# ntampellini/FIRECODE

Hardware: AMD Instinct MI355X
Metric: conformer-pair RMSD alignments/s (higher is better)
Workload: dtype f64

## Files before the change

firecode_amd/csrc/fc_kabsch.hip:

```cpp
#include <type_traits>

#include "fc_internal.h"
#include <vector>
#include "fc_kabsch_math.h"

#include <algorithm>
#include <cstdlib>

namespace fc {

__global__ void __launch_bounds__(256)
k_prep(const double *__restrict__ coords, int64_t N, int64_t A_all, const int32_t *__restrict__ sel,
       int64_t A, int center, int64_t Npad, double *__restrict__ Xs, double *__restrict__ G,
       double *__restrict__ Xa, unsigned long long *__restrict__ gmax_bits,
       const int32_t *__restrict__ conf_idx) {
  const int64_t n = (int64_t)blockIdx.x * blockDim.x + threadIdx.x;
  if (n >= Npad) return;
  for (int64_t a = A; a < ((A + 3) & ~(int64_t)3); ++a) {
    Xs[(a * 3 + 0) * Npad + n] = 0.0;
    Xs[(a * 3 + 1) * Npad + n] = 0.0;
    Xs[(a * 3 + 2) * Npad + n] = 0.0;
  }
  if (n >= N) {
    for (int64_t a = 0; a < A; ++a) {
// ... 430 lines not shown
    push_pairs(m, may, i, j, pairq, Q, counters, lane);
  }
}

__device__ __forceinline__ void flush_pairs_wave32(const uint32_t *__restrict__ sq_wave, int n_staged, unsigned i0, unsigned j0,
                                                   uint64_t *__restrict__ pairq, unsigned long long Q,
                                                   unsigned long long *__restrict__ counters, int lane) {
  if (n_staged == 0) return;
  unsigned long long base = 0;
  if (lane == 0) base = atomicAdd(&counters[6], (unsigned long long)n_staged);
  base = __shfl(base, 0);
  for (int idx = lane; idx < n_staged; idx += 64) {
    const uint32_t e = sq_wave[idx];
    const unsigned long long slot = base + (unsigned long long)idx;
    if (slot < Q) pairq[slot] = ((uint64_t)(i0 + (e >> 6)) << 32) | (uint64_t)(j0 + (e & 63u));
  }
}
template <int WCAP>
__device__ __forceinline__ void stage_pairs_wave32(uint64_t m, bool may, unsigned i, unsigned j, unsigned i0, unsigned j0,
                                                   uint32_t *__restrict__ sq_wave, int &n_staged,
                                                   uint64_t *__restrict__ pairq, unsigned long long Q,
                                                   unsigned long long *__restrict__ counters, int lane) {
  if (m == 0) return;
  const int n = (int)__popcll(m);
  if (n > WCAP) {
    push_pairs(m, may, i, j, pairq, Q, counters, lane);
    return;
  }
  if (n_staged + n > WCAP) {
    flush_pairs_wave32(sq_wave, n_staged, i0, j0, pairq, Q, counters, lane);
    n_staged = 0;
  }
  if (may) sq_wave[n_staged + (int)__popcll(m & ((1ull << lane) - 1ull))] = ((i - i0) << 6) | (j - j0);
  n_staged += n;
}

template <bool USE_LDS, int TI, int NW, bool ENANT = false>
__global__ void __launch_bounds__(NW * 64)
k_simbits_screen(const double *__restrict__ Xs, const double *__restrict__ G, int64_t N,
                 int64_t Npad, int A, double A_thr2, int IB, int64_t rank, int64_t world,
                 uint64_t *__restrict__ bits, int64_t W, uint32_t *__restrict__ cand,
                 unsigned long long *__restrict__ counters, uint64_t *__restrict__ pairq,
                 unsigned long long Q) {
  extern __shared__ double lds[];
  const int tid = threadIdx.x;
  const int lane = tid & 63;
  const int wv = __builtin_amdgcn_readfirstlane(tid >> 6);
  const int64_t jt = blockIdx.x;
  const int64_t lb = blockIdx.y;
  const int64_t gb = global_block(lb, rank, world);
  const int64_t i0 = gb * IB;
  if (i0 >= N) return;
  if (jt * 64 + 63 <= i0) return;
  const int64_t j = jt * 64 + lane;

  if (USE_LDS) {
    const int total = A * 3 * 64;
    for (int idx = tid; idx < total; idx += NW * 64) {
      const int ac = idx >> 6, l = idx & 63;
      lds[idx] = Xs[(int64_t)ac * Npad + jt * 64 + l];
    }
    __syncthreads();
  }
  const double Gq = G[j];
  const double *__restrict__ xq = Xs + jt * 64 + lane;

  for (int it = wv; it * TI < IB; it += NW) {
    const int64_t ib = i0 + (int64_t)it * TI;
    if (ib >= N) break;
    if (jt * 64 + 63 <= ib) break;
    double acc[TI][9];
#pragma unroll
    for (int k = 0; k < TI; ++k)
#pragma unroll
      for (int e = 0; e < 9; ++e) acc[k][e] = 0.0;

    const double *__restrict__ xp = Xs + ib;
#pragma unroll 2
    for (int a = 0; a < A; ++a) {
      double qx, qy, qz;
      if (USE_LDS) {
        qx = lds[(a * 3 + 0) * 64 + lane];
        qy = lds[(a * 3 + 1) * 64 + lane];
        qz = lds[(a * 3 + 2) * 64 + lane];
      } else {
        qx = xq[(int64_t)(a * 3 + 0) * Npad];
        qy = xq[(int64_t)(a * 3 + 1) * Npad];
        qz = xq[(int64_t)(a * 3 + 2) * Npad];
      }
      const double *__restrict__ px = xp + (int64_t)(a * 3 + 0) * Npad;
      const double *__restrict__ py = xp + (int64_t)(a * 3 + 1) * Npad;
      const double *__restrict__ pz = xp + (int64_t)(a * 3 + 2) * Npad;
#pragma unroll
      for (int k = 0; k < TI; ++k) {
        const double x = px[k], y = py[k], z = pz[k];
        acc[k][0] = fma(x, qx, acc[k][0]);
        acc[k][1] = fma(x, qy, acc[k][1]);
        acc[k][2] = fma(x, qz, acc[k][2]);
        acc[k][3] = fma(y, qx, acc[k][3]);
        acc[k][4] = fma(y, qy, acc[k][4]);
        acc[k][5] = fma(y, qz, acc[k][5]);
        acc[k][6] = fma(z, qx, acc[k][6]);
        acc[k][7] = fma(z, qy, acc[k][7]);
        acc[k][8] = fma(z, qz, acc[k][8]);
      }
    }
#pragma unroll
    for (int k = 0; k < TI; ++k) {
      const int64_t i = ib + k;
      const double Gp = G[i];
      bool may = kabsch_may_be_below<ENANT>(acc[k], Gp + Gq, A_thr2);
      may = may && (j > i) && (j < N) && (i < N);
      const uint64_t word = __ballot(may);
      push_pairs(word, may, (unsigned)i, (unsigned)j, pairq, Q, counters, lane);
      if (lane == 0 && i < N) {
        const int64_t lrow = (int64_t)(lb * IB) + (int64_t)it * TI + k;
        bits[lrow * W + jt] = word;
        if (word) {
          const unsigned long long slot = atomicAdd(&counters[4], 1ull);
          cand[slot] = (uint32_t)(lrow * W + jt);
        }
      }
    }
  }
}

typedef double d4_t __attribute__((ext_vector_type(4)));

template <int NW, int MODE = 0, int TC = 64, bool EIG = false, bool ENANT = false>
__global__ void __launch_bounds__(NW * 64, 2)
k_simbits_screen_mfma(const double *__restrict__ Xs, const double *__restrict__ G, int64_t N,
                      int64_t Npad, int A, double A_thr2, int IB, int64_t rank, int64_t world,
                      uint64_t *__restrict__ bits, int64_t W, uint32_t *__restrict__ cand,
                      unsigned long long *__restrict__ counters, uint64_t *__restrict__ pairq,
                      unsigned long long Q, const uint64_t *__restrict__ item_table, unsigned long long n_items,
                      double *__restrict__ rmsd_out = nullptr, const unsigned long long *__restrict__ gate = nullptr,
                      double *__restrict__ maxdev_out = nullptr) {
  static_assert(!EIG || MODE == 2, "EIG: the complete alignments");
  static_assert(!ENANT || MODE == 0, "ENANT: the screen only");
  constexpr bool VALUES = MODE != 0;
  constexpr int NT = MODE == 2 ? 1 : 2;
  static_assert(TC == 64 || ((TC == 32 || TC == 16) && MODE == 2), "column tiles: 64, or 32 / 16 for the complete alignments");
  constexpr int NU = (TC / 16) / NT;
  constexpr int KPR = TC == 64 ? 2 : 4;
  constexpr int SST = 2048 / TC;
  constexpr int CST = TC == 64 ? 256 : 128;
  auto koff = [](int sl) { return TC == 16 ? (sl >> 1) * 384 + (sl & 1) * 64 : sl * (12 * TC); };
  if (gate != nullptr && *gate == 0ull) return;
  extern __shared__ double lds[];
  const int tid = threadIdx.x;
  const int lane = tid & 63;
  const int wv = __builtin_amdgcn_readfirstlane(tid >> 6);
  const int KS = (A + 3) >> 2;
  double *__restrict__ ldsG = lds + (TC == 16 ? ((KS + 1) >> 1) * 384 : KS * 12 * TC);
  uint64_t *__restrict__ stageQ = reinterpret_cast<uint64_t *>(ldsG + TC + IB);
  uint32_t *__restrict__ stageW = reinterpret_cast<uint32_t *>(stageQ + kStagePairs);
  unsigned *__restrict__ stageN = reinterpret_cast<unsigned *>(stageW + kStageWords);
#ifdef FC_TIMELINE
  unsigned long long *tl = MODE == 2 ? reinterpret_cast<unsigned long long *>(bits) : reinterpret_cast<unsigned long long *>(rmsd_out);
  constexpr bool TL = MODE == 0 || MODE == 2;
#endif
  const unsigned long long b = blockIdx.x;
  if (b >= n_items) return;
#ifdef FC_TIMELINE
  if (TL && tl && tid == 0) {
    tl[(size_t)b * 4] = wall_clock64();
    tl[(size_t)b * 4 + 3] = b;
  }
#endif
  int64_t jt, lb;
  int it_first = 0, it_last = IB >> 4;
  if (item_table != nullptr) {
    const uint64_t it = item_table[b];
    lb = item_block(it);
    jt = item_tile(it);
    if constexpr (MODE == 2) it_last = (IB >> 4) * item_blocks(it);
    if (it & kItemFirstHalf) it_last = IB >> 5;
    if (it & kItemSecondHalf) it_first = IB >> 5;
  } else {
    const int64_t NT = Npad / TC;
    jt = (int64_t)(b % (unsigned long long)NT);
    lb = (int64_t)(b / (unsigned long long)NT);
  }
  const int64_t j0 = jt * TC;
  const int64_t i0 = global_block(lb, rank, world) * IB;
  if (i0 >= N) return;
  if (j0 + TC - 1 <= i0) return;
  uint32_t *__restrict__ sq32_wave = reinterpret_cast<uint32_t *>(stageQ) + wv * (kStagePairs * 2 / NW);
  int n_staged32 = 0;
  (void)sq32_wave;
  (void)n_staged32;

  {
    const int n_runs = TC == 64 ? KS * 6 : (TC == 32 ? KS * 3 : ((KS + 1) >> 1) * 3);
    const int cs_l = TC == 64 ? lane >> 4 : lane >> 5, k1_l = TC == 64 ? (lane >> 3) & 1 : (lane >> 3) & 3, c15_l = (lane & 7) * 2;
    for (int q = wv; q < n_runs; q += NW) {
      const int sc = TC == 64 ? q >> 1 : q, kh = TC == 64 ? q & 1 : 0;
      const int sg = sc / 3, c = sc - sg * 3;
      int a = sg * 4 + kh * 2 + k1_l;
      if (TC == 16) {
        a = (sg * 2 + cs_l) * 4 + k1_l;
        a = a < KS * 4 ? a : KS * 4 - 1;
      }
      const double *src = Xs + (int64_t)(a * 3 + c) * Npad + j0 + (TC == 16 ? 0 : cs_l * 16) + c15_l;
      __builtin_amdgcn_global_load_lds((const __attribute__((address_space(1))) void *)src,
                                       (__attribute__((address_space(3))) void *)(lds + q * 128), 16, 0, 0);
    }
    for (int idx = tid; idx < TC + IB; idx += NW * 64) {
      const int64_t g = idx < TC ? j0 + idx : i0 + (idx - TC);
      ldsG[idx] = g < Npad ? G[g] : 0.0;
    }
    if (tid < kStagePairs) stageQ[tid] = ~0ull;
    if (tid < kStageWords) stageW[tid] = ~0u;
    if (tid < 2) stageN[tid] = 0u;
    __syncthreads();
#ifdef FC_TIMELINE
    if (TL && tl && tid == 0) tl[(size_t)b * 4 + 1] = wall_clock64();
#endif
  }
  const int kq = lane >> 4, l15 = lane & 15;
  const int lcol = MODE == 2 ? 4 * (l15 & 3) + (l15 >> 2) : l15;
  const int boff = (kq / KPR) * 128 + (kq % KPR) * 16 + lcol;
  uint16_t *bits16 = reinterpret_cast<uint16_t *>(bits);

  double a0[3], a1[3], a2[3];
  int pre_it = -1;
  const int tpb = IB >> 4;
  auto tile_row = [&](int it_) -> int64_t {
    if constexpr (MODE == 2) {
      const int k = it_ / tpb;
      return global_block(lb + k, rank, world) * IB + (int64_t)(it_ - k * tpb) * 16;
    } else {
      return i0 + (int64_t)it_ * 16;
    }
  };
  auto row_offsets = [&](int it_, unsigned (&vo)[3]) {
    const int64_t ib_ = tile_row(it_);
#pragma unroll
    for (int c = 0; c < 3; ++c) vo[c] = (unsigned)(((int64_t)(kq * 3 + c) * Npad + ib_ + l15) * 8);
  };
  auto fetch_a_at = [&](double (&a)[3], unsigned (&vo)[3], int sx) {
    const int sl = sx < KS ? sx : KS - 1;
    const char *__restrict__ xs_s = reinterpret_cast<const char *>(Xs + (int64_t)sl * 12 * Npad);
#pragma unroll
    for (int c = 0; c < 3; ++c) {
      asm volatile("" : "+v"(vo[c]));
      a[c] = *reinterpret_cast<const double *>(xs_s + vo[c]);
    }
  };

  for (int it = it_first + wv; it < it_last; it += NW) {
    const int64_t ib = tile_row(it);
    if (ib >= N) break;
    if (j0 + TC - 1 <= ib) break;
    const int64_t lrow0 = lb * IB + (int64_t)it * 16;
    double Gp_row = 0.0;
    if constexpr (MODE == 2) Gp_row = G[ib + l15];
    (void)Gp_row;
    unsigned nz = 0;
    unsigned voff[3];
    row_offsets(it, voff);

#pragma unroll 1
    for (int half = 0; half < NU; ++half) {
      const int cs0 = half * NT;
      if (j0 + (cs0 + NT) * 16 - 1 <= ib) {
        if (!VALUES && lane < 16 && ib + lane < N) {
          bits16[((lrow0 + lane) * W + jt) * 4 + cs0] = 0;
          bits16[((lrow0 + lane) * W + jt) * 4 + cs0 + 1] = 0;
        }
        continue;
      }
      if constexpr (MODE == 2) {
        if (j0 + cs0 * 16 >= N) continue;
      }
      d4_t acc[NT][9];

      const double *__restrict__ lb0 = lds + cs0 * SST + boff;
      double b0[NT][3], b1[NT][3];
      const int KSe = KS;
      auto fetch_a = [&](double (&a)[3], int sx) {
        fetch_a_at(a, voff, sx);
      };
      auto fetch_b = [&](double (&b)[NT][3], int sx) {
        const int sl = sx < KS ? sx : KS - 1;
        const double *__restrict__ lb_s = lb0 + koff(sl);
#pragma unroll
        for (int t = 0; t < NT; ++t)
#pragma unroll
          for (int c = 0; c < 3; ++c) b[t][c] = lb_s[c * CST + t * SST];
      };
      auto mma = [&](const double (&a)[3], const double (&b)[NT][3], auto first_) {
        constexpr bool first = decltype(first_)::value;
#pragma unroll
        for (int x = 0; x < 3; ++x)
#pragma unroll
          for (int y = 0; y < 3; ++y)
#pragma unroll
            for (int t = 0; t < NT; ++t) {
              const d4_t c_in = first ? d4_t{0.0, 0.0, 0.0, 0.0} : acc[t][x * 3 + y];
              acc[t][x * 3 + y] = MODE == 2 ? __builtin_amdgcn_mfma_f64_16x16x4f64(b[t][y], a[x], c_in, 0, 0, 0)
                                            : __builtin_amdgcn_mfma_f64_16x16x4f64(a[x], b[t][y], c_in, 0, 0, 0);
            }
      };
      if (pre_it != it) {
        fetch_a_at(a0, voff, 0);
        fetch_a_at(a1, voff, 1);
        fetch_a_at(a2, voff, 2);
      }
      fetch_b(b0, 0);
      fetch_b(b1, 1);
#define FC_KSTEP(AX, BX, U)             \
  if (sgrp + (U) < KSe) {               \
    mma(AX, BX, std::false_type{});     \
    fetch_a(AX, sgrp + (U) + 3);        \
    fetch_b(BX, sgrp + (U) + 2);        \
  }
      mma(a0, b0, std::true_type{});
      fetch_a(a0, 3);
      fetch_b(b0, 2);
      for (int sgrp = 1; sgrp < KSe; sgrp += 6) {
        FC_KSTEP(a1, b1, 0)
        FC_KSTEP(a2, b0, 1)
        FC_KSTEP(a0, b1, 2)
        FC_KSTEP(a1, b0, 3)
        FC_KSTEP(a2, b1, 4)
        FC_KSTEP(a0, b0, 5)
      }
#undef FC_KSTEP
      {
        const bool same_tile = half < NU - 1 && !(MODE == 2 && j0 + (cs0 + NT) * 16 >= N);
        const int nit = same_tile ? it : it + NW;
        bool more = same_tile;
        if (!same_tile && nit < it_last) {
          const int64_t nib = tile_row(nit);
          more = nib < N && !(j0 + TC - 1 <= nib);
        }
        if (more) {
          unsigned vn[3];
          row_offsets(nit, vn);
          fetch_a_at(a0, vn, 0);
          fetch_a_at(a1, vn, 1);
          fetch_a_at(a2, vn, 2);
          pre_it = nit;
        } else {
          pre_it = -1;
        }
      }
      const int n32 = (int)N, ib32 = (int)ib;
#pragma unroll
      for (int t = 0; t < NT; ++t) {
        const int cs = cs0 + t;
        const int j = (int)j0 + cs * 16 + l15;
        const double Gq = ldsG[cs * 16 + l15];
        uint64_t mr[4] = {0, 0, 0, 0};
        if (MODE == 2) {
          const int i = ib32 + l15;
          const int jb = (int)j0 + cs * 16 + 4 * kq;
          const double Gp = Gp_row;
          double nR[4][9];
          bool ok4[4];
          double msdA4[4] = {0.0, 0.0, 0.0, 0.0};
          {
            double B4[4][9], GG[4], Q44[4][4], nq4[4], lam4[4];
#pragma unroll
            for (int r = 0; r < 4; ++r) {
              GG[r] = Gp + ldsG[cs * 16 + 4 * kq + r];
#pragma unroll
              for (int e = 0; e < 9; ++e) B4[r][e] = acc[t][e][r];
            }
            kabsch_quaternion_qcp_lean4(B4, GG, Q44, nq4, ok4, EIG ? lam4 : nullptr);
            if constexpr (EIG) {
              const double k_small = 2e-10 / (double)A;
#pragma unroll
              for (int r = 0; r < 4; ++r) {
                msdA4[r] = GG[r] - 2.0 * lam4[r];
                if (!(msdA4[r] > k_small * GG[r] * GG[r])) ok4[r] = false, msdA4[r] = 0.0;
              }
            }
#pragma unroll
            for (int r = 0; r < 4; ++r) {
              if (!ok4[r]) Q44[r][0] = 1.0, Q44[r][1] = 0.0, Q44[r][2] = 0.0, Q44[r][3] = 0.0, nq4[r] = 1.0;
              neg_rotation_from_raw_quaternion(Q44[r], nq4[r], nR[r]);
            }
          }
          typedef double d2_t __attribute__((ext_vector_type(2)));
          const double *__restrict__ qcol = lds + cs * SST + 4 * kq;
          const double *__restrict__ prow_u = Xs + ib;
          const unsigned l15u = (unsigned)l15;
          const int n_rounds = (A + 1) >> 1, n_groups = n_rounds >> 1;
          const bool odd_round = (n_rounds & 1) != 0;
          double ssq[4] = {0.0, 0.0, 0.0, 0.0}, mx[4] = {0.0, 0.0, 0.0, 0.0};
          const int64_t Npad3 = 3 * Npad;
          const double *__restrict__ pa0 = prow_u, *__restrict__ pa1 = prow_u + Npad, *__restrict__ pa2 = prow_u + 2 * Npad;
          const double *__restrict__ qg = qcol;
          auto load_pq = [&](auto u_, double (&P)[3], d2_t (&Qv)[3][2]) {
            constexpr int u = decltype(u_)::value;
            const double *__restrict__ ql = qg + (u / KPR) * 128 + (u % KPR) * 16;
#pragma unroll
            for (int c = 0; c < 3; ++c) {
              Qv[c][0] = *reinterpret_cast<const d2_t *>(ql + c * CST);
              Qv[c][1] = *reinterpret_cast<const d2_t *>(ql + c * CST + 2);
            }
            P[0] = pa0[l15u];
            P[1] = pa1[l15u];
            P[2] = pa2[l15u];
            pa0 += Npad3;
            pa1 += Npad3;
            pa2 += Npad3;
          };
          auto accumulate = [&](const double (&P)[3], const d2_t (&Qv)[3][2]) {
#pragma clang fp contract(fast)
#pragma unroll
            for (int r = 0; r < 4; ++r) {
              const double qx = Qv[0][r >> 1][r & 1], qy = Qv[1][r >> 1][r & 1], qz = Qv[2][r >> 1][r & 1];
              const double dx = fma(nR[r][0], qx, fma(nR[r][1], qy, fma(nR[r][2], qz, P[0])));
              const double dy = fma(nR[r][3], qx, fma(nR[r][4], qy, fma(nR[r][5], qz, P[1])));
              const double dz = fma(nR[r][6], qx, fma(nR[r][7], qy, fma(nR[r][8], qz, P[2])));
              const double s2 = fma(dz, dz, fma(dy, dy, dx * dx));
              if constexpr (!EIG) ssq[r] += s2;
              asm("v_max_f64 %0, %1, %2" : "=v"(mx[r]) : "v"(mx[r]), "v"(s2));
            }
          };
          using U0 = std::integral_constant<int, 0>;
          using U1 = std::integral_constant<int, 1>;
          using U2 = std::integral_constant<int, 2>;
          using U3 = std::integral_constant<int, 3>;
          double PA[3], PB[3];
          d2_t QA[3][2], QB[3][2];
          load_pq(U0{}, PA, QA);
          for (int g = 0; g < n_groups; ++g) {
            load_pq(U1{}, PB, QB);
            __builtin_amdgcn_sched_barrier(0);
            accumulate(PA, QA);
            __builtin_amdgcn_sched_barrier(0);
            load_pq(U2{}, PA, QA);
            __builtin_amdgcn_sched_barrier(0);
            accumulate(PB, QB);
            __builtin_amdgcn_sched_barrier(0);
            load_pq(U3{}, PB, QB);
            __builtin_amdgcn_sched_barrier(0);
            accumulate(PA, QA);
            __builtin_amdgcn_sched_barrier(0);
            qg = TC == 16 ? qcol + koff(g + 1) : qg + 12 * TC;
            if (g + 1 < n_groups || odd_round) load_pq(U0{}, PA, QA);
            __builtin_amdgcn_sched_barrier(0);
            accumulate(PB, QB);
            __builtin_amdgcn_sched_barrier(0);
          }
          if (odd_round) {
            load_pq(U1{}, PB, QB);
            __builtin_amdgcn_sched_barrier(0);
            accumulate(PA, QA);
            __builtin_amdgcn_sched_barrier(0);
            accumulate(PB, QB);
          }
          if constexpr (EIG) {
#pragma unroll
            for (int r = 0; r < 4; ++r) ssq[r] = msdA4[r];
          }
          const bool row_in = i < n32;
          double *__restrict__ ro = rmsd_out + (int64_t)i * N + jb;
          double *__restrict__ mo = maxdev_out + (int64_t)i * N + jb;
          const double invA = 1.0 / (double)A;
          if (row_in && jb > i && jb + 3 < n32 && ((((int64_t)i * N) & 1) == 0)) {
            *reinterpret_cast<d2_t *>(ro) = d2_t{fc_sqrt_nonneg(ssq[0] * invA), fc_sqrt_nonneg(ssq[1] * invA)};
            *reinterpret_cast<d2_t *>(ro + 2) = d2_t{fc_sqrt_nonneg(ssq[2] * invA), fc_sqrt_nonneg(ssq[3] * invA)};
            *reinterpret_cast<d2_t *>(mo) = d2_t{fc_sqrt_nonneg(mx[0]), fc_sqrt_nonneg(mx[1])};
            *reinterpret_cast<d2_t *>(mo + 2) = d2_t{fc_sqrt_nonneg(mx[2]), fc_sqrt_nonneg(mx[3])};
          } else {
#pragma unroll
            for (int r = 0; r < 4; ++r) {
              const int j = jb + r;
              if (row_in && j >= i && j < n32) {
                ro[r] = j == i ? 0.0 : fc_sqrt_nonneg(ssq[r] * invA);
                mo[r] = j == i ? 0.0 : fc_sqrt_nonneg(mx[r]);
              }
            }
          }
#pragma unroll
          for (int r = 0; r < 4; ++r) {
            const int j = jb + r;
            const bool redo = row_in && (j > i) && (j < n32) && !ok4[r];
            stage_pairs(__ballot(redo), redo, (unsigned)i, (unsigned)j, stageQ, stageN, pairq, Q, counters, lane);
          }
          continue;
        }
#pragma unroll
        for (int r = 0; r < 4; ++r) {
          const int i = ib32 + kq + 4 * r;
          const double Gp = ldsG[TC + it * 16 + kq + 4 * r];
          double B9[9];
#pragma unroll
          for (int e = 0; e < 9; ++e) B9[e] = acc[t][e][r];
          if (VALUES) {
            double slope;
            const double lam = kabsch_lambda_max(B9, Gp + Gq, &slope);
            const double msdA = (Gp + Gq) - 2.0 * lam;
            const bool in = (j > i) && (j < n32) && (i < n32);
            if (in) rmsd_out[(int64_t)i * N + j] = sqrt(fmax(msdA, 0.0) / (double)A);
            const bool redo = in && (msdA < A_thr2 || !kabsch_lambda_is_sharp(lam, slope, (double)A, msdA));
            stage_pairs(__ballot(redo), redo, (unsigned)i, (unsigned)j, stageQ, stageN, pairq, Q, counters, lane);
            continue;
          }
          bool may = kabsch_may_be_below<ENANT>(B9, Gp + Gq, A_thr2);
          may = may && (j > i) && (j < n32) && (i < n32);
          mr[r] = __ballot(may);
          if constexpr (MODE == 0)
            stage_pairs_wave32<kStagePairs * 2 / NW>(mr[r], may, (unsigned)i, (unsigned)j, (unsigned)i0, (unsigned)j0, sq32_wave,
                                                     n_staged32, pairq, Q, counters, lane);
          else
            stage_pairs(mr[r], may, (unsigned)i, (unsigned)j, stageQ, stageN, pairq, Q, counters, lane);
        }
        if (!VALUES && lane < 16 && ib32 + lane < n32) {
          const int rr = lane >> 2;
          const uint64_t mine = rr == 0 ? mr[0] : rr == 1 ? mr[1] : rr == 2 ? mr[2] : mr[3];
          const unsigned piece = (unsigned)((mine >> (16 * (lane & 3))) & 0xffffull);
          bits16[((lrow0 + lane) * W + jt) * 4 + cs] = (uint16_t)piece;
          nz |= piece;
        }
      }
    }
    if (!VALUES) {
#ifndef FC_ABLATE_PUSH
      const bool has = lane < 16 && nz != 0;
      const uint64_t mw = __ballot(has);
      if (mw != 0) {
        const unsigned n = (unsigned)__popcll(mw);
        const uint32_t word = (uint32_t)((lrow0 + lane) * W + jt);
        unsigned base = 0;
        if (lane == 0) base = atomicAdd(stageN + 1, n);
        base = (unsigned)__builtin_amdgcn_readfirstlane((int)base);
        const unsigned rank_in = (unsigned)__popcll(mw & ((1ull << lane) - 1ull));
        if (base + n <= (unsigned)kStageWords) {
          if (has) stageW[base + rank_in] = word;
        } else {
          unsigned long long gbase = 0;
// ... 2567 lines not shown
```

firecode_amd/csrc/fc_kabsch_math.h:

```cpp
#pragma once
#include <hip/hip_runtime.h>

namespace fc {

template <int P, int Q>
__host__ __device__ __forceinline__ void jacobi_rot(double (&a)[4][4], double (&v)[4][4], bool late) {
  const double apq = a[P][Q];
  const double g = 100.0 * fabs(apq);
  const double app = a[P][P], aqq = a[Q][Q];
  if (late && (fabs(app) + g == fabs(app)) && (fabs(aqq) + g == fabs(aqq))) {
    a[P][Q] = 0.0;
    a[Q][P] = 0.0;
    return;
  }
  if (apq == 0.0) return;
  const double h = aqq - app;
  double t;
  if (fabs(h) + g == fabs(h)) {
    t = apq / h;
  } else {
    const double theta = 0.5 * h / apq;
    t = 1.0 / (fabs(theta) + sqrt(1.0 + theta * theta));
    if (theta < 0.0) t = -t;
  }
// ... 322 lines not shown
  y = y * (1.5 - hx * y * y);
  y = y * (1.5 - hx * y * y);
  return y;
}

__host__ __device__ __forceinline__ double fc_sqrt_nonneg(double x) {
#if defined(__HIP_DEVICE_COMPILE__)
#pragma clang fp contract(fast)
  const double y = __builtin_amdgcn_rsq(x);
  double g = x * y, h = 0.5 * y;
  const double r = fma(-h, g, 0.5);
  g = fma(g, r, g);
  h = fma(h, r, h);
  const double d = fma(-g, g, x);
  g = fma(d, h, g);
  const double d2 = fma(-g, g, x);
  g = fma(d2, h, g);
  return x > 0.0 ? g : 0.0;
#else
  return sqrt(x);
#endif
}

__host__ __device__ __forceinline__ bool kabsch_quaternion_qcp(const double (&B)[9], double GpGq, double (&Q)[4],
                                                               int *iterations = nullptr) {
#pragma clang fp contract(fast)
  const double Sxx = B[0], Sxy = B[3], Sxz = B[6];
  const double Syx = B[1], Syy = B[4], Syz = B[7];
  const double Szx = B[2], Szy = B[5], Szz = B[8];
  const double n2 = Sxx * Sxx + Sxy * Sxy + Sxz * Sxz + Syx * Syx + Syy * Syy + Syz * Syz +
                    Szx * Szx + Szy * Szy + Szz * Szz;
  const double c00 = Syy * Szz - Syz * Szy, c01 = Syz * Szx - Syx * Szz, c02 = Syx * Szy - Syy * Szx;
  const double c10 = Sxz * Szy - Sxy * Szz, c11 = Sxx * Szz - Sxz * Szx, c12 = Sxy * Szx - Sxx * Szy;
  const double c20 = Sxy * Syz - Sxz * Syy, c21 = Sxz * Syx - Sxx * Syz, c22 = Sxx * Syy - Sxy * Syx;
  const double detB = Sxx * c00 + Sxy * c01 + Sxz * c02;
  const double e2 = c00 * c00 + c01 * c01 + c02 * c02 + c10 * c10 + c11 * c11 + c12 * c12 +
                    c20 * c20 + c21 * c21 + c22 * c22;
  const double C2 = -2.0 * n2, C1 = -8.0 * detB, C0 = n2 * n2 - 4.0 * e2;
  double x = 0.5 * GpGq;
  int it = 0;
  for (; it < 64; ++it) {
    const double x2 = x * x;
    const double b = (x2 + C2) * x;
    const double a = b + C1;
    const double den = 2.0 * x2 * x + b + a;
    if (den == 0.0) break;
    const double delta = (a * x + C0) * fc_rcp_approx(den);
    x -= delta;
    if (fabs(delta) <= 1e-9 * fabs(x)) break;
  }
  if (iterations) *iterations = it + 1;
  const double lam = x;
  const double m00 = (Sxx + Syy + Szz) - lam, m01 = Syz - Szy, m02 = Szx - Sxz, m03 = Sxy - Syx;
  const double m11 = (Sxx - Syy - Szz) - lam, m12 = Sxy + Syx, m13 = Szx + Sxz;
  const double m22 = (-Sxx + Syy - Szz) - lam, m23 = Syz + Szy;
  const double m33 = (-Sxx - Syy + Szz) - lam;
  const double L01 = m02 * m13 - m12 * m03, L02 = m02 * m23 - m22 * m03, L03 = m02 * m33 - m23 * m03;
  const double L12 = m12 * m23 - m22 * m13, L13 = m12 * m33 - m23 * m13, L23 = m22 * m33 - m23 * m23;
  const double U01 = m00 * m11 - m01 * m01, U02 = m00 * m12 - m02 * m01, U03 = m00 * m13 - m03 * m01;
  const double U12 = m01 * m12 - m02 * m11, U13 = m01 * m13 - m03 * m11, U23 = m02 * m13 - m03 * m12;
  (void)U23;
  const double a00 = m11 * L23 - m12 * L13 + m13 * L12;
  const double a01 = -(m01 * L23 - m12 * L03 + m13 * L02);
  const double a02 = m01 * L13 - m11 * L03 + m13 * L01;
  const double a03 = -(m01 * L12 - m11 * L02 + m12 * L01);
  const double a11 = m00 * L23 - m02 * L03 + m03 * L02;
  const double a12 = -(m00 * L13 - m01 * L03 + m03 * L01);
  const double a13 = m00 * L12 - m01 * L02 + m02 * L01;
  const double a22 = m03 * U13 - m13 * U03 + m33 * U01;
  const double a23 = -(m03 * U12 - m13 * U02 + m23 * U01);
  const double a33 = m02 * U12 - m12 * U02 + m22 * U01;
  double q0 = a00, q1 = a01, q2 = a02, q3 = a03, best = fabs(a00);
  if (fabs(a11) > best) { best = fabs(a11); q0 = a01; q1 = a11; q2 = a12; q3 = a13; }
  if (fabs(a22) > best) { best = fabs(a22); q0 = a02; q1 = a12; q2 = a22; q3 = a23; }
  if (fabs(a33) > best) { best = fabs(a33); q0 = a03; q1 = a13; q2 = a23; q3 = a33; }
  const double scale = fabs(lam) + fabs(Sxx) + fabs(Syy) + fabs(Szz) + fabs(m01) + fabs(m02) + fabs(m03) +
                       fabs(m12) + fabs(m13) + fabs(m23);
  const double nq = q0 * q0 + q1 * q1 + q2 * q2 + q3 * q3;
  if (!(best > 2e-3 * scale * scale * scale) || !(nq > 0.0)) return false;
  const double nrm = fc_rsqrt(nq);
  q0 *= nrm; q1 *= nrm; q2 *= nrm; q3 *= nrm;
  const double r0 = m00 * q0 + m01 * q1 + m02 * q2 + m03 * q3;
  const double r1 = m01 * q0 + m11 * q1 + m12 * q2 + m13 * q3;
  const double r2 = m02 * q0 + m12 * q1 + m22 * q2 + m23 * q3;
  const double r3 = m03 * q0 + m13 * q1 + m23 * q2 + m33 * q3;
  if (!(fmax(fmax(fabs(r0), fabs(r1)), fmax(fabs(r2), fabs(r3))) <= 1e-12 * scale)) return false;
  Q[0] = q0; Q[1] = q1; Q[2] = q2; Q[3] = q3;
  return true;
}

struct QcpLeanPoly {
  double C2, C1, C0, n2;
};
__host__ __device__ __forceinline__ QcpLeanPoly qcp_lean_polynomial(const double (&B)[9]) {
#pragma clang fp contract(fast)
  const double Sxx = B[0], Sxy = B[3], Sxz = B[6];
  const double Syx = B[1], Syy = B[4], Syz = B[7];
  const double Szx = B[2], Szy = B[5], Szz = B[8];
  const double n2 = Sxx * Sxx + Sxy * Sxy + Sxz * Sxz + Syx * Syx + Syy * Syy + Syz * Syz +
                    Szx * Szx + Szy * Szy + Szz * Szz;
  const double c00 = Syy * Szz - Syz * Szy, c01 = Syz * Szx - Syx * Szz, c02 = Syx * Szy - Syy * Szx;
  const double c10 = Sxz * Szy - Sxy * Szz, c11 = Sxx * Szz - Sxz * Szx, c12 = Sxy * Szx - Sxx * Szy;
  const double c20 = Sxy * Syz - Sxz * Syy, c21 = Sxz * Syx - Sxx * Syz, c22 = Sxx * Syy - Sxy * Syx;
  const double detB = Sxx * c00 + Sxy * c01 + Sxz * c02;
  const double e2 = c00 * c00 + c01 * c01 + c02 * c02 + c10 * c10 + c11 * c11 + c12 * c12 +
                    c20 * c20 + c21 * c21 + c22 * c22;
  return QcpLeanPoly{-2.0 * n2, -8.0 * detB, n2 * n2 - 4.0 * e2, n2};
}
__host__ __device__ __forceinline__ bool qcp_lean_step(const QcpLeanPoly &P, double &x, double &delta) {
#pragma clang fp contract(fast)
  const double x2 = x * x;
  const double b = (x2 + P.C2) * x;
  const double a = b + P.C1;
  const double den = 2.0 * x2 * x + b + a;
  delta = (a * x + P.C0) * fc_rcp_approx(den);
  x -= delta;
  return fabs(delta) > 1e-9 * fabs(x);
}
__host__ __device__ __forceinline__ bool qcp_lean_quaternion_raw(const double (&B)[9], const QcpLeanPoly &P, double lam,
                                                                 double delta, double (&Q)[4], double &nq_out) {
#pragma clang fp contract(fast)
  const double Sxx = B[0], Sxy = B[3], Sxz = B[6];
  const double Syx = B[1], Syy = B[4], Syz = B[7];
  const double Szx = B[2], Szy = B[5], Szz = B[8];
  const bool converged = fabs(delta) <= 1e-9 * fabs(lam);
  const double m00 = (Sxx + Syy + Szz) - lam, m01 = Syz - Szy, m02 = Szx - Sxz, m03 = Sxy - Syx;
  const double m11 = (Sxx - Syy - Szz) - lam, m12 = Sxy + Syx, m13 = Szx + Sxz;
  const double m22 = (-Sxx + Syy - Szz) - lam, m23 = Syz + Szy;
  const double m33 = (-Sxx - Syy + Szz) - lam;
  const double L01 = m02 * m13 - m12 * m03, L02 = m02 * m23 - m22 * m03, L03 = m02 * m33 - m23 * m03;
  const double L12 = m12 * m23 - m22 * m13, L13 = m12 * m33 - m23 * m13, L23 = m22 * m33 - m23 * m23;
  const double U01 = m00 * m11 - m01 * m01, U02 = m00 * m12 - m02 * m01, U03 = m00 * m13 - m03 * m01;
  const double U12 = m01 * m12 - m02 * m11, U13 = m01 * m13 - m03 * m11;
  const double a00 = m11 * L23 - m12 * L13 + m13 * L12;
  const double a01 = -(m01 * L23 - m12 * L03 + m13 * L02);
  const double a02 = m01 * L13 - m11 * L03 + m13 * L01;
  const double a03 = -(m01 * L12 - m11 * L02 + m12 * L01);
  const double a11 = m00 * L23 - m02 * L03 + m03 * L02;
  const double a12 = -(m00 * L13 - m01 * L03 + m03 * L01);
  const double a13 = m00 * L12 - m01 * L02 + m02 * L01;
  const double a22 = m03 * U13 - m13 * U03 + m33 * U01;
  const double a23 = -(m03 * U12 - m13 * U02 + m23 * U01);
  const double a33 = m02 * U12 - m12 * U02 + m22 * U01;
  double q0 = a00, q1 = a01, q2 = a02, q3 = a03, best = fabs(a00);
  if (fabs(a11) > best) { best = fabs(a11); q0 = a01; q1 = a11; q2 = a12; q3 = a13; }
  if (fabs(a22) > best) { best = fabs(a22); q0 = a02; q1 = a12; q2 = a22; q3 = a23; }
  if (fabs(a33) > best) { best = fabs(a33); q0 = a03; q1 = a13; q2 = a23; q3 = a33; }
  const double nq = q0 * q0 + q1 * q1 + q2 * q2 + q3 * q3;
  const bool simple = best * best > (2e-3 * 27.0) * (2e-3 * 27.0) * (P.n2 * P.n2) * P.n2;
  Q[0] = q0; Q[1] = q1; Q[2] = q2; Q[3] = q3;
  nq_out = nq;
  return converged && simple && nq > 0.0;
}
__host__ __device__ __forceinline__ bool qcp_lean_quaternion(const double (&B)[9], const QcpLeanPoly &P, double lam,
                                                             double delta, double (&Q)[4]) {
  double nq;
  const bool ok = qcp_lean_quaternion_raw(B, P, lam, delta, Q, nq);
  const double nrm = fc_rsqrt(nq);
  Q[0] *= nrm; Q[1] *= nrm; Q[2] *= nrm; Q[3] *= nrm;
  return ok;
}

__host__ __device__ __forceinline__ bool kabsch_quaternion_qcp_lean(const double (&B)[9], double GpGq, double (&Q)[4],
                                                                    int *iterations = nullptr) {
  const QcpLeanPoly P = qcp_lean_polynomial(B);
  double x = 0.5 * GpGq, delta = 0.0;
  int it = 0;
  for (; it < 64; ++it) {
    const bool moving = qcp_lean_step(P, x, delta);
#if defined(__HIP_DEVICE_COMPILE__)
    if (__builtin_amdgcn_ballot_w64(moving) == 0ull) break;
#else
    if (!moving) break;
#endif
  }
  if (iterations) *iterations = it + 1;
  return qcp_lean_quaternion(B, P, x, delta, Q);
}

__host__ __device__ __forceinline__ void kabsch_quaternion_qcp_lean4(const double (&B)[4][9], const double (&GpGq)[4],
                                                                     double (&Q)[4][4], double (&nq)[4], bool (&ok)[4],
                                                                     double *lam_out = nullptr) {
  QcpLeanPoly P[4];
  double x[4], delta[4] = {0.0, 0.0, 0.0, 0.0};
#pragma unroll
  for (int r = 0; r < 4; ++r) {
    P[r] = qcp_lean_polynomial(B[r]);
    x[r] = 0.5 * GpGq[r];
  }
  for (int it = 0; it < 64; ++it) {
    bool moving = false;
#pragma unroll
    for (int r = 0; r < 4; ++r) moving |= qcp_lean_step(P[r], x[r], delta[r]);
#if defined(__HIP_DEVICE_COMPILE__)
    if (__builtin_amdgcn_ballot_w64(moving) == 0ull) break;
#else
    if (!moving) break;
#endif
  }
#pragma unroll
  for (int r = 0; r < 4; ++r) ok[r] = qcp_lean_quaternion_raw(B[r], P[r], x[r], delta[r], Q[r], nq[r]);
  if (lam_out != nullptr) {
#pragma unroll
    for (int r = 0; r < 4; ++r) lam_out[r] = x[r];
  }
}

__host__ __device__ __forceinline__ void rotation_from_quaternion(const double (&Q)[4], double (&R)[9]) {
#pragma clang fp contract(fast)
  const double q0 = Q[0], q1 = Q[1], q2 = Q[2], q3 = Q[3];
  R[0] = q0 * q0 + q1 * q1 - q2 * q2 - q3 * q3;
  R[1] = 2.0 * (q1 * q2 - q0 * q3);
  R[2] = 2.0 * (q1 * q3 + q0 * q2);
  R[3] = 2.0 * (q1 * q2 + q0 * q3);
  R[4] = q0 * q0 - q1 * q1 + q2 * q2 - q3 * q3;
  R[5] = 2.0 * (q2 * q3 - q0 * q1);
  R[6] = 2.0 * (q1 * q3 - q0 * q2);
  R[7] = 2.0 * (q2 * q3 + q0 * q1);
  R[8] = q0 * q0 - q1 * q1 - q2 * q2 + q3 * q3;
}

__host__ __device__ __forceinline__ void neg_rotation_from_quaternion(const double (&Q)[4], double (&R)[9]) {
#pragma clang fp contract(fast)
  const double q0 = Q[0], q1 = Q[1], q2 = Q[2], q3 = Q[3];
  R[0] = q2 * q2 + q3 * q3 - q0 * q0 - q1 * q1;
  R[1] = -2.0 * (q1 * q2 - q0 * q3);
  R[2] = -2.0 * (q1 * q3 + q0 * q2);
  R[3] = -2.0 * (q1 * q2 + q0 * q3);
  R[4] = q1 * q1 + q3 * q3 - q0 * q0 - q2 * q2;
  R[5] = -2.0 * (q2 * q3 - q0 * q1);
  R[6] = -2.0 * (q1 * q3 - q0 * q2);
  R[7] = -2.0 * (q2 * q3 + q0 * q1);
  R[8] = q1 * q1 + q2 * q2 - q0 * q0 - q3 * q3;
}

__host__ __device__ __forceinline__ void neg_rotation_from_raw_quaternion(const double (&Q)[4], double nq, double (&R)[9]) {
#pragma clang fp contract(fast)
  const double q0 = Q[0], q1 = Q[1], q2 = Q[2], q3 = Q[3];
  double inv = fc_rcp_approx(nq);
  inv = fma(fma(-nq, inv, 1.0), inv, inv);
  inv = fma(fma(-nq, inv, 1.0), inv, inv);
  const double t = inv + inv;
  const double p11 = q1 * q1, p22 = q2 * q2;
  R[0] = fma(t, fma(q3, q3, p22), -1.0);
  R[4] = fma(t, fma(q3, q3, p11), -1.0);
  R[8] = fma(t, p11 + p22, -1.0);
  const double a12 = q1 * q2, a13 = q1 * q3, a23 = q2 * q3;
  R[1] = t * fma(q0, q3, -a12);
  R[3] = -t * fma(q0, q3, a12);
  R[2] = -t * fma(q0, q2, a13);
  R[6] = t * fma(q0, q2, -a13);
  R[5] = t * fma(q0, q1, -a23);
  R[7] = -t * fma(q0, q1, a23);
}

}
```

firecode_amd/csrc/fc_tuning.h:

```cpp
#pragma once

#if !defined(FC_TUNING_BUILD) &&                                                                                             \
    (defined(FC_TIMELINE) || defined(FC_H2_TIMELINE) || defined(FC_RB_TIMELINE) || defined(FC_TFD_STAMPS) || defined(FC_TFD_STAMPS_SMALL) || defined(FC_H2_ABLATE_K) ||   \
     defined(FC_H2_ABLATE_ROWS) || defined(FC_H2_ABLATE_POLY) || defined(FC_F32_ABLATE_K) || defined(FC_F32_ABLATE_POLY) ||  \
     defined(FC_ABLATE_PUSH) || defined(FC_ABLATE_STAGE) || defined(FC_ABLATE_OVERFLOW) || defined(FC_ABLATE_REDO) ||         \
     defined(FC_RB_NOSTAGE) || defined(FC_RB_NOPASS1) || defined(FC_RB_NOPASS2) || defined(FC_RB_NOJACOBI) ||                \
     defined(FC_RB_NOCOMPUTE) || defined(FC_RB_ROWS_FROM_LDS) || defined(FC_RB_SAMEROW) || defined(FC_RB_WPS) ||              \
     defined(FC_RB_AHEAD) || defined(FC_RB_CHUNK) || defined(FC_H2_WGS) || defined(FC_F32_WGS) || defined(FC_REFINE_ROUNDS) || defined(FC_STAGE_PAIRS_F32) || defined(FC_TS_WGS) || defined(FC_TS_TURN))
#error "a tuning switch (FC_*TIMELINE / FC_*ABLATE* / FC_RB_* / FC_TFD_STAMPS ...) without -DFC_TUNING_BUILD: see fc_tuning.h"
#endif

#ifdef __cplusplus
namespace fc {
constexpr int64_t kDiverseLanes8MaxN = 10000;
}
#endif
```

Before: 20.24 billion.

## Build rotation from QCP adjugate directly and handle K-tail atoms with scalar FMAs

In the complete-alignment mode, the rotation matrix is now built straight from the adjugate of the shifted QCP key matrix, with a Newton-refined reciprocal. This replaces the quaternion extraction, normalization and quaternion-to-rotation conversion. Separately, when the atom count leaves a remainder of 1 or 2 in the last 4-wide K step, that final MFMA step is skipped and those atoms are added to the correlation matrix with scalar FMAs. This avoids a mostly zero-padded MFMA slice at the cost of extra loads and FMAs. Both paths can be disabled with tuning switches, and the adjugate path changes how degenerate cases fall back to the identity.

```diff
diff --git a/firecode_amd/csrc/fc_kabsch.hip b/firecode_amd/csrc/fc_kabsch.hip
--- a/firecode_amd/csrc/fc_kabsch.hip
+++ b/firecode_amd/csrc/fc_kabsch.hip
@@ -606,6 +606,11 @@
   const int lane = tid & 63;
   const int wv = __builtin_amdgcn_readfirstlane(tid >> 6);
   const int KS = (A + 3) >> 2;
+#ifndef FC_COMPLETE_NO_KTAIL
+  const int ktail = (MODE == 2 && A >= 4 && ((A & 3) == 1 || (A & 3) == 2)) ? (A & 3) : 0;
+#else
+  const int ktail = 0;
+#endif
   double *__restrict__ ldsG = lds + (TC == 16 ? ((KS + 1) >> 1) * 384 : KS * 12 * TC);
   uint64_t *__restrict__ stageQ = reinterpret_cast<uint64_t *>(ldsG + TC + IB);
   uint32_t *__restrict__ stageW = reinterpret_cast<uint32_t *>(stageQ + kStagePairs);
@@ -732,7 +737,7 @@
 
       const double *__restrict__ lb0 = lds + cs0 * SST + boff;
       double b0[NT][3], b1[NT][3];
-      const int KSe = KS;
+      const int KSe = ktail != 0 ? KS - 1 : KS;
       auto fetch_a = [&](double (&a)[3], int sx) {
         fetch_a_at(a, voff, sx);
       };
@@ -761,6 +766,19 @@
         fetch_a_at(a0, voff, 0);
         fetch_a_at(a1, voff, 1);
         fetch_a_at(a2, voff, 2);
+      }
+      double pt[2][3] = {{0.0, 0.0, 0.0}, {0.0, 0.0, 0.0}};
+      if constexpr (MODE == 2) {
+        if (ktail != 0) {
+          const double *__restrict__ pt_u = Xs + (int64_t)KSe * 12 * Npad + ib;
+          const unsigned l15t = (unsigned)l15;
+#pragma unroll
+          for (int c = 0; c < 3; ++c) pt[0][c] = pt_u[(int64_t)c * Npad + l15t];
+          if (ktail > 1) {
+#pragma unroll
+            for (int c = 0; c < 3; ++c) pt[1][c] = pt_u[(int64_t)(3 + c) * Npad + l15t];
+          }
+        }
       }
       fetch_b(b0, 0);
       fetch_b(b1, 1);
@@ -816,13 +834,51 @@
           bool ok4[4];
           double msdA4[4] = {0.0, 0.0, 0.0, 0.0};
           {
-            double B4[4][9], GG[4], Q44[4][4], nq4[4], lam4[4];
+            double B4[4][9], GG[4];
 #pragma unroll
             for (int r = 0; r < 4; ++r) {
               GG[r] = Gp + ldsG[cs * 16 + 4 * kq + r];
 #pragma unroll
               for (int e = 0; e < 9; ++e) B4[r][e] = acc[t][e][r];
             }
+            if (ktail != 0) {
+              typedef double d2t_t __attribute__((ext_vector_type(2)));
+              const double *__restrict__ qt = lds + cs * SST + 4 * kq + koff(KSe);
+              auto add_atom = [&](auto u_) {
+                constexpr int u = decltype(u_)::value;
+                const double *__restrict__ ql = qt + (u / KPR) * 128 + (u % KPR) * 16;
+                d2t_t qv[3][2];
+#pragma unroll
+                for (int c = 0; c < 3; ++c) {
+                  qv[c][0] = *reinterpret_cast<const d2t_t *>(ql + c * CST);
+                  qv[c][1] = *reinterpret_cast<const d2t_t *>(ql + c * CST + 2);
+                }
+#pragma unroll
+                for (int r = 0; r < 4; ++r)
+#pragma unroll
+                  for (int x = 0; x < 3; ++x)
+#pragma unroll
+                    for (int y = 0; y < 3; ++y) B4[r][x * 3 + y] = fma(pt[u][x], qv[y][r >> 1][r & 1], B4[r][x * 3 + y]);
+              };
+              add_atom(std::integral_constant<int, 0>{});
+              if (ktail > 1) add_atom(std::integral_constant<int, 1>{});
+            }
+#ifndef FC_COMPLETE_NO_ADJUGATE
+            QcpLeanPoly P4[4];
+            double lam4[4], delta4[4];
+            qcp_lean_newton4(B4, GG, P4, lam4, delta4);
+#pragma unroll
+            for (int r = 0; r < 4; ++r) {
+              bool wanted = true;
+              if constexpr (EIG) {
+                const double k_small = 2e-10 / (double)A;
+                msdA4[r] = GG[r] - 2.0 * lam4[r];
+                if (!(msdA4[r] > k_small * GG[r] * GG[r])) wanted = false, msdA4[r] = 0.0;
+              }
+              ok4[r] = qcp_lean_neg_rotation_from_adjugate(B4[r], P4[r], lam4[r], delta4[r], wanted, nR[r]);
+            }
+#else
+            double Q44[4][4], nq4[4], lam4[4];
             kabsch_quaternion_qcp_lean4(B4, GG, Q44, nq4, ok4, EIG ? lam4 : nullptr);
             if constexpr (EIG) {
               const double k_small = 2e-10 / (double)A;
@@ -837,6 +893,7 @@
               if (!ok4[r]) Q44[r][0] = 1.0, Q44[r][1] = 0.0, Q44[r][2] = 0.0, Q44[r][3] = 0.0, nq4[r] = 1.0;
               neg_rotation_from_raw_quaternion(Q44[r], nq4[r], nR[r]);
             }
+#endif
           }
           typedef double d2_t __attribute__((ext_vector_type(2)));
           const double *__restrict__ qcol = lds + cs * SST + 4 * kq;
diff --git a/firecode_amd/csrc/fc_kabsch_math.h b/firecode_amd/csrc/fc_kabsch_math.h
--- a/firecode_amd/csrc/fc_kabsch_math.h
+++ b/firecode_amd/csrc/fc_kabsch_math.h
@@ -498,6 +498,52 @@
   nq_out = nq;
   return converged && simple && nq > 0.0;
 }
+__host__ __device__ __forceinline__ bool qcp_lean_neg_rotation_from_adjugate(const double (&B)[9], const QcpLeanPoly &P,
+                                                                             double lam_in, double delta, bool wanted,
+                                                                             double (&R)[9]) {
+#pragma clang fp contract(fast)
+  const double Sxx = B[0], Sxy = B[3], Sxz = B[6];
+  const double Syx = B[1], Syy = B[4], Syz = B[7];
+  const double Szx = B[2], Szy = B[5], Szz = B[8];
+  const bool converged = fabs(delta) <= 1e-9 * fabs(lam_in);
+  const double lam = converged ? lam_in : 0.0;
+  const double m00 = (Sxx + Syy + Szz) - lam, m01 = Syz - Szy, m02 = Szx - Sxz, m03 = Sxy - Syx;
+  const double m11 = (Sxx - Syy - Szz) - lam, m12 = Sxy + Syx, m13 = Szx + Sxz;
+  const double m22 = (-Sxx + Syy - Szz) - lam, m23 = Syz + Szy;
+  const double m33 = (-Sxx - Syy + Szz) - lam;
+  const double L01 = m02 * m13 - m12 * m03, L02 = m02 * m23 - m22 * m03, L03 = m02 * m33 - m23 * m03;
+  const double L12 = m12 * m23 - m22 * m13, L13 = m12 * m33 - m23 * m13, L23 = m22 * m33 - m23 * m23;
+  const double U01 = m00 * m11 - m01 * m01, U02 = m00 * m12 - m02 * m01, U03 = m00 * m13 - m03 * m01;
+  const double U12 = m01 * m12 - m02 * m11, U13 = m01 * m13 - m03 * m11;
+  const double a00 = m11 * L23 - m12 * L13 + m13 * L12;
+  const double a01 = -(m01 * L23 - m12 * L03 + m13 * L02);
+  const double a02 = m01 * L13 - m11 * L03 + m13 * L01;
+  const double a03 = -(m01 * L12 - m11 * L02 + m12 * L01);
+  const double a11 = m00 * L23 - m02 * L03 + m03 * L02;
+  const double a12 = -(m00 * L13 - m01 * L03 + m03 * L01);
+  const double a13 = m00 * L12 - m01 * L02 + m02 * L01;
+  const double a22 = m03 * U13 - m13 * U03 + m33 * U01;
+  const double a23 = -(m03 * U12 - m13 * U02 + m23 * U01);
+  const double a33 = m02 * U12 - m12 * U02 + m22 * U01;
+  const double d01 = a00 + a11, d12 = a11 + a22, d23 = a22 + a33, d13 = a11 + a33;
+  const double tr = d01 + d23;
+  const bool simple = tr < 0.0 && tr * tr > (8e-3 * 27.0) * (8e-3 * 27.0) * (P.n2 * P.n2) * P.n2;
+  const bool ok = converged && simple && wanted;
+  double inv = fc_rcp_approx(tr);
+  inv = fma(fma(-tr, inv, 1.0), inv, inv);
+  inv = fma(fma(-tr, inv, 1.0), inv, inv);
+  const double t = ok ? inv + inv : 0.0;
+  R[0] = fma(t, d23, -1.0);
+  R[4] = fma(t, d13, -1.0);
+  R[8] = fma(t, d12, -1.0);
+  R[1] = t * (a03 - a12);
+  R[3] = -t * (a03 + a12);
+  R[2] = -t * (a02 + a13);
+  R[6] = t * (a02 - a13);
+  R[5] = t * (a01 - a23);
+  R[7] = -t * (a01 + a23);
+  return ok;
+}
 __host__ __device__ __forceinline__ bool qcp_lean_quaternion(const double (&B)[9], const QcpLeanPoly &P, double lam,
                                                              double delta, double (&Q)[4]) {
   double nq;
@@ -524,15 +570,13 @@
   return qcp_lean_quaternion(B, P, x, delta, Q);
 }
 
-__host__ __device__ __forceinline__ void kabsch_quaternion_qcp_lean4(const double (&B)[4][9], const double (&GpGq)[4],
-                                                                     double (&Q)[4][4], double (&nq)[4], bool (&ok)[4],
-                                                                     double *lam_out = nullptr) {
-  QcpLeanPoly P[4];
-  double x[4], delta[4] = {0.0, 0.0, 0.0, 0.0};
+__host__ __device__ __forceinline__ void qcp_lean_newton4(const double (&B)[4][9], const double (&GpGq)[4],
+                                                          QcpLeanPoly (&P)[4], double (&x)[4], double (&delta)[4]) {
 #pragma unroll
   for (int r = 0; r < 4; ++r) {
     P[r] = qcp_lean_polynomial(B[r]);
     x[r] = 0.5 * GpGq[r];
+    delta[r] = 0.0;
   }
   for (int it = 0; it < 64; ++it) {
     bool moving = false;
@@ -544,6 +588,14 @@
     if (!moving) break;
 #endif
   }
+}
+
+__host__ __device__ __forceinline__ void kabsch_quaternion_qcp_lean4(const double (&B)[4][9], const double (&GpGq)[4],
+                                                                     double (&Q)[4][4], double (&nq)[4], bool (&ok)[4],
+                                                                     double *lam_out = nullptr) {
+  QcpLeanPoly P[4];
+  double x[4], delta[4];
+  qcp_lean_newton4(B, GpGq, P, x, delta);
 #pragma unroll
   for (int r = 0; r < 4; ++r) ok[r] = qcp_lean_quaternion_raw(B[r], P[r], x[r], delta[r], Q[r], nq[r]);
   if (lam_out != nullptr) {
diff --git a/firecode_amd/csrc/fc_tuning.h b/firecode_amd/csrc/fc_tuning.h
--- a/firecode_amd/csrc/fc_tuning.h
+++ b/firecode_amd/csrc/fc_tuning.h
@@ -6,7 +6,8 @@
      defined(FC_ABLATE_PUSH) || defined(FC_ABLATE_STAGE) || defined(FC_ABLATE_OVERFLOW) || defined(FC_ABLATE_REDO) ||         \
      defined(FC_RB_NOSTAGE) || defined(FC_RB_NOPASS1) || defined(FC_RB_NOPASS2) || defined(FC_RB_NOJACOBI) ||                \
      defined(FC_RB_NOCOMPUTE) || defined(FC_RB_ROWS_FROM_LDS) || defined(FC_RB_SAMEROW) || defined(FC_RB_WPS) ||              \
-     defined(FC_RB_AHEAD) || defined(FC_RB_CHUNK) || defined(FC_H2_WGS) || defined(FC_F32_WGS) || defined(FC_REFINE_ROUNDS) || defined(FC_STAGE_PAIRS_F32) || defined(FC_TS_WGS) || defined(FC_TS_TURN))
+     defined(FC_RB_AHEAD) || defined(FC_RB_CHUNK) || defined(FC_H2_WGS) || defined(FC_F32_WGS) || defined(FC_REFINE_ROUNDS) || defined(FC_STAGE_PAIRS_F32) || defined(FC_TS_WGS) || defined(FC_TS_TURN) ||   \
+     defined(FC_COMPLETE_NO_ADJUGATE) || defined(FC_COMPLETE_NO_KTAIL))
 #error "a tuning switch (FC_*TIMELINE / FC_*ABLATE* / FC_RB_* / FC_TFD_STAMPS ...) without -DFC_TUNING_BUILD: see fc_tuning.h"
 #endif
 
```

Result: faster. 20.52 billion, median of 6 (+1.4%).
